# yerfor/Real3DPortrait

Hardware: NVIDIA H100
Metric: rendered frames/sec @512^2 (64^2 NeRF, 48 samples/ray) (higher is better)
Workload: dtype f32 render (decoder GEMMs: split-fp16 operands on wgmma, f32 accumulate, f32-grade results); SR f16 operands / f32 accumulate (wgmma)

## Files before the change

real3dportrait_b200/csrc/sr_tc.cu:

```cuda
#include "common.cuh"
#include "tc_prims.cuh"
#include <mutex>
#include <vector>
#include <type_traits>
#include <stdlib.h>

#ifndef R3DP_TC_DEBUG_TIMING
#define R3DP_TC_DEBUG_TIMING 0
#endif
namespace r3dp {
namespace tc {

constexpr int BM = 128, BN = 128, BK = 64;
constexpr float kSplitWeightScale = 1024.0f;


struct Taps {
    int n;
    int dy[9], dx[9], widx[9];
};
enum Mode { kStoreAct = 0, kStoreRaw = 1, kToRgbFinal = 2 };
struct ConvArgs {
    Taps taps;
    int k_chunks;
// ... 21 lines not shown
    Taps2 taps;
    int rows, oy_off, ox_off;
};
enum Mode2 { kActRgb = 3 };
struct Conv2Args {
    Phase2 ph[4];
    int n_phases, k_chunks, tiles_x, row_groups, n_blocks, n_images, total_units;
    int w_shared, mode;
    __half* out; int out_H, out_W, out_C, oy_mul, ox_mul;
    const float* bias; const float* wrgb; const float* brgb; const float* img_prev; float* img_out; int img_H, img_W;
    float act_slope, act_gain;
    int skip_same_res;
    const __half* residual;
    int out_clamp;
    uint8_t* img_out_u8;
    int split;
    int lo_off;
    int phase_mix;
    float acc_scale;
    unsigned long long* debug;
};


__device__ __forceinline__ float upsampled_skip(const float* __restrict__ ip, int h, int w, int Y, int X) {
    const float k4[4] = {0.25f, 0.75f, 0.75f, 0.25f};
    float acc = 0.f;
#pragma unroll
    for (int u = 0; u < 4; ++u) {
        const int zy = Y + u - 2;
        if (zy < 0 || (zy & 1) || (zy >> 1) >= h) continue;
        float rowv = 0.f;
#pragma unroll
        for (int v = 0; v < 4; ++v) {
            const int zx = X + v - 2;
            if (zx < 0 || (zx & 1) || (zx >> 1) >= w) continue;
            rowv = fmaf(k4[v], __ldg(ip + (size_t)(zy >> 1) * w + (zx >> 1)), rowv);
        }
        acc = fmaf(k4[u], rowv, acc);
    }
    return acc;
}

__device__ __forceinline__ float upsampled_skip_bf(const float* __restrict__ ip, int h, int w, int Y, int X) {
    const int y0 = (Y - 1) >> 1, x0 = (X - 1) >> 1;
    const float ky0 = (y0 >= 0 && y0 < h) ? ((Y & 1) ? 0.75f : 0.25f) : 0.f, ky1 = (y0 + 1 < h) ? ((Y & 1) ? 0.25f : 0.75f) : 0.f;
    const float kx0 = (x0 >= 0 && x0 < w) ? ((X & 1) ? 0.75f : 0.25f) : 0.f, kx1 = (x0 + 1 < w) ? ((X & 1) ? 0.25f : 0.75f) : 0.f;
    const int ya = min(max(y0, 0), h - 1), yb = min(y0 + 1, h - 1), xa = min(max(x0, 0), w - 1), xb = min(x0 + 1, w - 1);
    const float v00 = __ldg(ip + (size_t)ya * w + xa), v01 = __ldg(ip + (size_t)ya * w + xb);
    const float v10 = __ldg(ip + (size_t)yb * w + xa), v11 = __ldg(ip + (size_t)yb * w + xb);
    const float r0 = fmaf(kx1, v01, fmaf(kx0, v00, 0.f)), r1 = fmaf(kx1, v11, fmaf(kx0, v10, 0.f));
    return fmaf(ky1, r1, fmaf(ky0, r0, 0.f));
}

__device__ __forceinline__ float2 fma2(float2 a, float2 b, float2 c) { return make_float2(__fmaf_rn(a.x, b.x, c.x), __fmaf_rn(a.y, b.y, c.y)); }
__device__ __forceinline__ float2 mul2(float2 a, float2 b) { return make_float2(__fmul_rn(a.x, b.x), __fmul_rn(a.y, b.y)); }
__device__ __forceinline__ float2 add2(float2 a, float2 b) { return make_float2(__fadd_rn(a.x, b.x), __fadd_rn(a.y, b.y)); }

__device__ __forceinline__ uint4 pack_half8(const float* f) {
    __half2 h0 = __floats2half2_rn(f[0], f[1]), h1 = __floats2half2_rn(f[2], f[3]);
    __half2 h2 = __floats2half2_rn(f[4], f[5]), h3 = __floats2half2_rn(f[6], f[7]);
    uint4 pk;
    pk.x = *reinterpret_cast<uint32_t*>(&h0); pk.y = *reinterpret_cast<uint32_t*>(&h1);
    pk.z = *reinterpret_cast<uint32_t*>(&h2); pk.w = *reinterpret_cast<uint32_t*>(&h3);
    return pk;
}

__device__ __forceinline__ void store_half32(__half* dst, const float* f) {
    uint4* d4 = reinterpret_cast<uint4*>(dst);
#pragma unroll
    for (int v = 0; v < 4; ++v) {
        __half2 h0 = __floats2half2_rn(f[8 * v + 0], f[8 * v + 1]), h1 = __floats2half2_rn(f[8 * v + 2], f[8 * v + 3]);
        __half2 h2 = __floats2half2_rn(f[8 * v + 4], f[8 * v + 5]), h3 = __floats2half2_rn(f[8 * v + 6], f[8 * v + 7]);
        uint4 pk;
        pk.x = *reinterpret_cast<uint32_t*>(&h0); pk.y = *reinterpret_cast<uint32_t*>(&h1);
        pk.z = *reinterpret_cast<uint32_t*>(&h2); pk.w = *reinterpret_cast<uint32_t*>(&h3);
        d4[v] = pk;
    }
}

constexpr int kThreads3 = 384;
constexpr int B3_BYTES = BN * BK * 2;
constexpr int kStageRow = BN + 8;
template <int R> struct Cfg3 {
    static constexpr int NA = 4, NB = 4;
    static constexpr int TAIL = 8192;
    static constexpr int STAGE = 8 * 32 * 64;
    static constexpr int ACC = BM * kStageRow * 4;
    static constexpr int SMEM = NA * A2_SLOT + NB * B3_BYTES + 1024 + TAIL + STAGE + ACC;
};

template <int R, bool SPLIT>
__global__ void __launch_bounds__(kThreads3, 1) conv_tc3_kernel(const __grid_constant__ CUtensorMap tmA,
                                                               const __grid_constant__ CUtensorMap tmB, const Conv2Args a) {
    using C = Cfg3<R>;
    extern __shared__ uint8_t smem_raw[];
    uint8_t* smem = align_smem_1024(smem_raw);
    uint8_t* a_ring = smem;
    uint8_t* b_ring = smem + C::NA * A2_SLOT;
    uint8_t* tail = b_ring + C::NB * B3_BYTES;
    uint64_t* a_full = reinterpret_cast<uint64_t*>(tail);
    uint64_t* a_empty = a_full + C::NA;
    uint64_t* b_full = a_empty + C::NA;
    uint64_t* b_empty = b_full + C::NB;
    float* s_bias = reinterpret_cast<float*>(tail + 512);
    float* s_wrgb = s_bias + 256;
    float* s_part = s_wrgb + 768;
    uint4* s_stage = reinterpret_cast<uint4*>(tail + C::TAIL);
    float* s_acc = reinterpret_cast<float*>(tail + C::TAIL + C::STAGE);

    const int warp = threadIdx.x >> 5, lane = threadIdx.x & 31;
    const int units_per_image = a.n_phases * a.row_groups * a.tiles_x;

    if (threadIdx.x == 0) {
        for (int i = 0; i < C::NA; ++i) { mbar_init(&a_full[i], 1); mbar_init(&a_empty[i], 256); }
        for (int i = 0; i < C::NB; ++i) { mbar_init(&b_full[i], 1); mbar_init(&b_empty[i], 256); }
        asm volatile("fence.mbarrier_init.release.cluster;" ::: "memory");
        asm volatile("prefetch.tensormap [%0];" ::"l"(&tmA) : "memory");
        asm volatile("prefetch.tensormap [%0];" ::"l"(&tmB) : "memory");
    }
    if (warp >= 4) {
        const int t = threadIdx.x - 128;
        for (int e = t; e < a.n_blocks * BN && e < 256; e += 256) s_bias[e] = a.bias ? a.bias[e] : 0.f;
    }
    __syncthreads();

    const bool mix = a.phase_mix && a.n_phases > 1 && (a.tiles_x & 1) == 0;
    auto decode = [&](int unit, int& n, int& ph, int& row0, int& col0) {
        n = unit / units_per_image; int r = unit - n * units_per_image;
        const int xb = r % a.tiles_x; r /= a.tiles_x;
        int rg;
        if (mix) { rg = r / a.n_phases; ph = (r - rg * a.n_phases + rg) % a.n_phases; }
        else { rg = r % a.row_groups; ph = r / a.row_groups; }
        row0 = rg * R; col0 = xb * BM;
    };

    if (warp < 4) {
        if (warp == 0 && lane == 0) {
            uint32_t aq = 0, bq = 0;
            for (int unit = blockIdx.x; unit < a.total_units; unit += gridDim.x) {
                int n, ph, row0, col0; decode(unit, n, ph, row0, col0);
                const Taps2& tp = a.ph[ph].taps;
                const int DY = tp.ngroups;
                const int wn = a.w_shared ? 0 : n;
                const int K3 = SPLIT ? 3 * a.k_chunks : a.k_chunks;
                for (int nblk = 0; nblk < a.n_blocks; ++nblk)
                    for (int kq = 0; kq < K3; ++kq) {
                        const int kc = kq < 2 * a.k_chunks ? kq : kq - 2 * a.k_chunks;
                        const int kb = kq < a.k_chunks ? kq : kq - a.k_chunks;
                        for (int d = 0; d < DY; ++d) {
                            const int s_lo = d == 0 ? 0 : R - 1 + d, s_hi = R - 1 + d;
                            for (int s = s_lo; s <= s_hi; ++s, ++aq) {
                                const int slot = aq % C::NA;
                                mbar_wait(&a_empty[slot], ((aq / C::NA) & 1) ^ 1);
                                mbar_expect_tx(&a_full[slot], A2_BYTES);
                                tma_load_4d(a_ring + slot * A2_SLOT, &tmA, &a_full[slot], kc * BK, col0 - 1, row0 + tp.dy_min + s, n);
                            }
                            for (int t = tp.gstart[d]; t < tp.gstart[d + 1]; ++t, ++bq) {
                                const int slot = bq % C::NB;
                                mbar_wait(&b_empty[slot], ((bq / C::NB) & 1) ^ 1);
                                mbar_expect_tx(&b_full[slot], B3_BYTES);
                                tma_load_4d(b_ring + slot * B3_BYTES, &tmB, &b_full[slot], kb * BK, nblk * BN, tp.widx[t], wn);
                            }
                        }
                    }
            }
        }
    } else {
        const int wg = (warp >> 2) - 1;
        const int q = warp & 3, m = q * 32 + lane;
        const int cg = wg;
        const bool want_rgb = (a.mode == kToRgbFinal) || (a.mode == kActRgb);
        const int CW = a.n_blocks * BN;
        float brgb[3] = {0.f, 0.f, 0.f};
        if (want_rgb) { brgb[0] = a.brgb[0]; brgb[1] = a.brgb[1]; brgb[2] = a.brgb[2]; }
        int n_loaded = -1;
        uint32_t aq = 0, bq = 0;
        int pend_b = -1; uint32_t pend_a0 = 0, pend_an = 0;
        auto release_pending = [&]() {
            if (pend_b >= 0) mbar_arrive(&b_empty[pend_b]);
            for (uint32_t s = 0; s < pend_an; ++s) mbar_arrive(&a_empty[(pend_a0 + s) % C::NA]);
            pend_b = -1; pend_an = 0;
        };
        float acc[R][64];
        for (int unit = blockIdx.x; unit < a.total_units; unit += gridDim.x) {
            int n, ph, row0, col0; decode(unit, n, ph, row0, col0);
            const Phase2& P = a.ph[ph];
            const Taps2& tp = P.taps;
            const int DY = tp.ngroups, NS = R + DY - 1;
            const int wn = a.w_shared ? 0 : n;
            if (want_rgb && wn != n_loaded) {
                asm volatile("bar.sync 1, 256;" ::: "memory");
                for (int e = threadIdx.x - 128; e < 3 * CW; e += 256) s_wrgb[e] = a.wrgb[(size_t)wn * 3 * CW + e];
                asm volatile("bar.sync 1, 256;" ::: "memory");
                n_loaded = wn;
            }
            const int gcol = col0 + m, X = gcol * a.ox_mul + P.ox_off;
            float2 rgb2[R][3];
#pragma unroll
            for (int j = 0; j < R; ++j) { rgb2[j][0] = make_float2(0.f, 0.f); rgb2[j][1] = make_float2(0.f, 0.f); rgb2[j][2] = make_float2(0.f, 0.f); }
            float skipv[R][3];
#pragma unroll
            for (int j = 0; j < R; ++j) { skipv[j][0] = 0.f; skipv[j][1] = 0.f; skipv[j][2] = 0.f; }
            if (want_rgb && cg == 1 && a.img_prev) {
                if (a.skip_same_res) {
                    const int Xc = min(X, a.img_W - 1);
#pragma unroll
                    for (int j = 0; j < R; ++j) {
                        const int Yc = min((row0 + j) * a.oy_mul + P.oy_off, a.img_H - 1);
#pragma unroll
                        for (int c = 0; c < 3; ++c) skipv[j][c] = __ldg(a.img_prev + (((size_t)n * 3 + c) * a.img_H + Yc) * a.img_W + Xc);
                    }
                } else {
                    const int h = a.img_H / 2, w = a.img_W / 2;
                    const int x0 = (X - 1) >> 1;
                    const float kx0 = (x0 >= 0 && x0 < w) ? ((X & 1) ? 0.75f : 0.25f) : 0.f, kx1 = (x0 + 1 < w) ? ((X & 1) ? 0.25f : 0.75f) : 0.f;
                    const int xa = min(max(x0, 0), w - 1), xb = min(max(x0 + 1, 0), w - 1);
#pragma unroll
                    for (int j = 0; j < R; ++j) {
                        const int Y = (row0 + j) * a.oy_mul + P.oy_off, y0 = (Y - 1) >> 1;
                        const float ky0 = (y0 >= 0 && y0 < h) ? ((Y & 1) ? 0.75f : 0.25f) : 0.f;
                        const float ky1 = (y0 + 1 < h) ? ((Y & 1) ? 0.25f : 0.75f) : 0.f;
                        const int ya = min(max(y0, 0), h - 1), yb = min(max(y0 + 1, 0), h - 1);
#pragma unroll
                        for (int c = 0; c < 3; ++c) {
                            const float* ip = a.img_prev + ((size_t)n * 3 + c) * h * w;
                            const float v0 = __ldg(ip + ya * w + xa), v1 = __ldg(ip + ya * w + xb), v2 = __ldg(ip + yb * w + xa), v3 = __ldg(ip + yb * w + xb);
                            const float r0 = fmaf(kx1, v1, fmaf(kx0, v0, 0.f)), r1 = fmaf(kx1, v3, fmaf(kx0, v2, 0.f));
                            skipv[j][c] = fmaf(ky1, r1, fmaf(ky0, r0, 0.f));
                        }
                    }
                }
            }
            for (int nblk = 0; nblk < a.n_blocks; ++nblk) {
                const int K3 = SPLIT ? 3 * a.k_chunks : a.k_chunks;
                for (int kc = 0; kc < K3; ++kc) {
                    const uint32_t a_base = aq;
                    for (int d = 0; d < DY; ++d) {
                        const int s_lo = d == 0 ? 0 : R - 1 + d, s_hi = R - 1 + d;
                        for (int s = s_lo; s <= s_hi; ++s, ++aq) mbar_wait(&a_full[aq % C::NA], (aq / C::NA) & 1);
                        for (int t = tp.gstart[d]; t < tp.gstart[d + 1]; ++t, ++bq) {
                            const int bslot = bq % C::NB;
                            mbar_wait(&b_full[bslot], (bq / C::NB) & 1);
                            const uint64_t db = gmma_desc_sw128(smem_u32(b_ring + bslot * B3_BYTES));
                            const int sh = tp.shift[t];
                            const uint32_t first = (uint32_t)(kc | t);
                            uint64_t da[R];
#pragma unroll
                            for (int j = 0; j < R; ++j) da[j] = gmma_desc_sw128(smem_u32(a_ring + ((a_base + j + d) % C::NA) * A2_SLOT) + 128 * (64 * wg + sh));
                            wg_fence();
#pragma unroll
                            for (int k = 0; k < BK / 16; ++k) {
#pragma unroll
                                for (int j = 0; j < R; ++j) wgmma_m64n128k16(acc[j], da[j] + (uint64_t)(2 * k), db + (uint64_t)(2 * k), first | (uint32_t)k);
                            }
                            wg_commit();
                            wg_wait<1>();
                            release_pending();
                            pend_b = bslot;
                        }
                        if (d < DY - 1) { pend_a0 = a_base + d; pend_an = 1; }
                        else { pend_a0 = a_base + DY - 1; pend_an = (uint32_t)(NS - (DY - 1)); }
                    }
                }
                wg_wait<0>();
#pragma unroll
                for (int j = 0; j < R; ++j) wg_fence_acc<64>(acc[j]);
                release_pending();
#pragma unroll
                for (int j = 0; j < R; ++j) {
#pragma unroll
                    for (int i = 0; i < 64; i += 2)
                        *reinterpret_cast<float2*>(s_acc + (64 * wg + acc_row(i)) * kStageRow + acc_col(i)) = make_float2(acc[j][i], acc[j][i + 1]);
                    asm volatile("bar.sync 4, 256;" ::: "memory");
                    const int row = row0 + j;
                    const int Y = row * a.oy_mul + P.oy_off;
                    const bool row_ok = (row < P.rows) && (Y < a.out_H);
                    const bool in_img = row_ok && (X < a.out_W);
#pragma unroll 1
                    for (int c0 = cg * (BN / 2); c0 < (cg + 1) * (BN / 2); c0 += 32) {
                        float2 f2[16];
                        const float4* src = reinterpret_cast<const float4*>(s_acc + m * kStageRow + c0);
                        const float2 sc2 = make_float2(a.acc_scale, a.acc_scale);
#pragma unroll
                        for (int i = 0; i < 8; ++i) { const float4 v = src[i]; f2[2 * i] = make_float2(v.x, v.y); f2[2 * i + 1] = make_float2(v.z, v.w); }
                        if (a.mode == kStoreRaw) {
                            if (SPLIT) {
#pragma unroll
                                for (int i = 0; i < 16; ++i) f2[i] = mul2(f2[i], sc2);
                            }
                        } else {
                            const float2* b2 = reinterpret_cast<const float2*>(s_bias + nblk * BN + c0);
                            const float2 sl2 = make_float2(a.act_slope, a.act_slope), g2 = make_float2(a.act_gain, a.act_gain);
#pragma unroll
                            for (int i = 0; i < 16; ++i) {
                                const float2 v = SPLIT ? fma2(f2[i], sc2, b2[i]) : add2(f2[i], b2[i]);
                                const float2 t = mul2(v, sl2);
                                f2[i] = mul2(make_float2(fmaxf(v.x, t.x), fmaxf(v.y, t.y)), g2);
                            }
                        }
                        const float* f = reinterpret_cast<const float*>(f2);
                        if (a.mode != kToRgbFinal) {
                            uint4* st = s_stage + (warp - 4) * 128;
                            const int sw = (lane >> 1) & 3;
                            constexpr int passes = SPLIT ? 2 : 1;
#pragma unroll
                            for (int pass = 0; pass < passes; ++pass) {
                                if (pass == 0) {
#pragma unroll
                                    for (int v = 0; v < 4; ++v) st[lane * 4 + (v ^ sw)] = pack_half8(f + 8 * v);
                                } else {
#pragma unroll
                                    for (int v = 0; v < 4; ++v) {
                                        float lo[8];
#pragma unroll
                                        for (int e = 0; e < 8; ++e) lo[e] = f[8 * v + e] - __half2float(__float2half_rn(f[8 * v + e]));
                                        st[lane * 4 + (v ^ sw)] = pack_half8(lo);
                                    }
                                }
                                __syncwarp();
#pragma unroll
                                for (int i = 0; i < 4; ++i) {
                                    const int p = i * 8 + (lane >> 2), cch = lane & 3;
                                    uint4 pk = st[p * 4 + (cch ^ ((p >> 1) & 3))];
                                    const int Xp = (col0 + q * 32 + p) * a.ox_mul + P.ox_off;
                                    if (row_ok && Xp < a.out_W) {
                                        const size_t eo = ((size_t)n * a.out_H + Y) * a.out_W * a.out_C + nblk * BN + (size_t)Xp * a.out_C + c0 + cch * 8 + pass * a.lo_off;
                                        if (a.residual) {
                                            const uint4 rv = __ldg(reinterpret_cast<const uint4*>(a.residual + eo));
                                            __half2* ph = reinterpret_cast<__half2*>(&pk); const __half2* rh = reinterpret_cast<const __half2*>(&rv);
#pragma unroll
                                            for (int e = 0; e < 4; ++e) { const float2 x = __half22float2(ph[e]), r = __half22float2(rh[e]); ph[e] = __floats2half2_rn(x.x + r.x, x.y + r.y); }
                                        }
                                        *reinterpret_cast<uint4*>(a.out + eo) = pk;
                                    }
                                }
                                __syncwarp();
                            }
                        }
                        if (want_rgb) {
#pragma unroll
                            for (int c = 0; c < 3; ++c) {
                                const float4* w4 = reinterpret_cast<const float4*>(s_wrgb + c * CW + nblk * BN + c0);
                                float2 accr = rgb2[j][c];
#pragma unroll
                                for (int j4 = 0; j4 < 8; ++j4) {
                                    const float4 w = w4[j4];
                                    accr = fma2(f2[2 * j4], make_float2(w.x, w.y), accr);
                                    accr = fma2(f2[2 * j4 + 1], make_float2(w.z, w.w), accr);
                                }
                                rgb2[j][c] = accr;
                            }
                        }
                    }
                    if (want_rgb && nblk == a.n_blocks - 1) {
                        if (cg == 1) {
#pragma unroll
                            for (int c = 0; c < 3; ++c) s_part[(j * BM + m) * 3 + c] = (rgb2[j][c].x + rgb2[j][c].y) + skipv[j][c];
                        }
                        asm volatile("bar.sync 2, 256;" ::: "memory");
                        if (cg == 0) {
#pragma unroll
                            for (int c = 0; c < 3; ++c) rgb2[j][c].x = (rgb2[j][c].x + rgb2[j][c].y) + s_part[(j * BM + m) * 3 + c];
                        }
                        asm volatile("bar.sync 3, 256;" ::: "memory");
                    }
                    if (want_rgb && nblk == a.n_blocks - 1 && in_img && cg == 0) {
#pragma unroll
                        for (int c = 0; c < 3; ++c) {
                            float v = rgb2[j][c].x + brgb[c];
                            if (a.out_clamp) v = fminf(fmaxf(v, -1.0f), 1.0f);
                            if (a.img_out_u8)
                                a.img_out_u8[(((size_t)n * a.img_H + Y) * a.img_W + X) * 3 + c] =
                                    (uint8_t)(int)__fmul_rn(__fmul_rn(__fadd_rn(v, 1.0f), 0.5f), 255.0f);
                            else
                                a.img_out[(((size_t)n * 3 + c) * a.img_H + Y) * a.img_W + X] = v;
                        }
                    }
                    asm volatile("bar.sync 5, 256;" ::: "memory");
                }
            }
        }
    }
}

__device__ __forceinline__ void split_half(float v, __half& hi, __half& lo) {
    hi = __float2half_rn(v);
    lo = __float2half_rn(v - __half2float(hi));
}

__global__ void pack_weights_kernel(const float* __restrict__ wf, int Nw, int O, int I, int Ip, int split, __half* __restrict__ out) {
    const long long idx = (long long)blockIdx.x * blockDim.x + threadIdx.x;
    const long long total = (long long)Nw * 9 * O * Ip;
    if (idx >= total) return;
    const int i = (int)(idx % Ip); const int o = (int)((idx / Ip) % O); const int t = (int)((idx / ((long long)Ip * O)) % 9);
    const int nw = (int)(idx / ((long long)Ip * O * 9));
    const float v = i < I ? wf[(((size_t)nw * O + o) * I + i) * 9 + t] : 0.f;
    if (!split) { out[idx] = __float2half_rn(v); return; }
    __half hi, lo;
    split_half(v * kSplitWeightScale, hi, lo);
    const size_t row = (idx / Ip) * (size_t)(2 * Ip);
    out[row + i] = hi; out[row + Ip + i] = lo;
}

__global__ void resize_to_nhwc_f16_kernel(const float* __restrict__ x, int N, int C, int h, int w, int size, int Cp, int split, __half* __restrict__ y) {
    const long long idx = (long long)blockIdx.x * blockDim.x + threadIdx.x;
    if (idx >= (long long)N * size * size * Cp) return;
    const int c = (int)(idx % Cp); const int ox = (int)((idx / Cp) % size); const int oy = (int)((idx / ((long long)Cp * size)) % size);
    const int n = (int)(idx / ((long long)Cp * size * size));
    float v = 0.f;
    if (c < C) {
        const float sy = fmaxf(((float)oy + 0.5f) * ((float)h / (float)size) - 0.5f, 0.f);
        const float sx = fmaxf(((float)ox + 0.5f) * ((float)w / (float)size) - 0.5f, 0.f);
        const int y0 = min((int)sy, h - 1), x0 = min((int)sx, w - 1), y1 = min(y0 + 1, h - 1), x1 = min(x0 + 1, w - 1);
        const float ty = sy - (float)y0, tx = sx - (float)x0;
        const float* p = x + ((size_t)n * C + c) * h * w;
        const float r0 = p[y0 * w + x0] * (1.f - ty) + p[y1 * w + x0] * ty;
        const float r1 = p[y0 * w + x1] * (1.f - ty) + p[y1 * w + x1] * ty;
        v = r0 * (1.f - tx) + r1 * tx;
    }
    if (!split) { y[idx] = __float2half_rn(v); return; }
    __half hi, lo;
    split_half(v, hi, lo);
    const size_t pix = (idx / Cp) * (size_t)(2 * Cp);
    y[pix + c] = hi; y[pix + Cp + c] = lo;
}

constexpr int kEdgeRows = 16, kEdgeRowsSplit = 16, kEdgeCo = 32;
__global__ void __launch_bounds__(256) upconv_edge_kernel(const __half* __restrict__ x, const __half* __restrict__ wp, int H, int W, int Cp, int O,
                                                          int w_shared, __half* __restrict__ yb) {
    extern __shared__ __align__(16) uint8_t edge_smem[];
    __half* s_x = reinterpret_cast<__half*>(edge_smem);
// ... 255 lines not shown
        if (cudaGetDriverEntryPoint("cuTensorMapEncodeTiled", &p, cudaEnableDefault, &q) == cudaSuccess && q == cudaDriverEntryPointSuccess)
            fn = reinterpret_cast<EncodeTiledFn>(p);
    });
    return fn;
}

static int make_map_4d_box(CUtensorMap* m, const void* ptr, uint64_t d0, uint64_t d1, uint64_t d2, uint64_t d3, uint32_t box1);
static int make_map_4d(CUtensorMap* m, const void* ptr, uint64_t d0, uint64_t d1, uint64_t d2, uint64_t d3, uint32_t box1) {
    return make_map_4d_box(m, ptr, d0, d1, d2, d3, box1);
}
static int make_map_4d_box(CUtensorMap* m, const void* ptr, uint64_t d0, uint64_t d1, uint64_t d2, uint64_t d3, uint32_t box1) {
    EncodeTiledFn fn = encode_fn();
    R3DP_REQUIRE(fn != nullptr, "cuTensorMapEncodeTiled is not available from the driver");
    cuuint64_t dims[4] = {d0, d1, d2, d3};
    cuuint64_t strides[3] = {d0 * 2, d0 * d1 * 2, d0 * d1 * d2 * 2};
    cuuint32_t box[4] = {64, box1, 1, 1};
    cuuint32_t estr[4] = {1, 1, 1, 1};
    CUresult r = fn(m, CU_TENSOR_MAP_DATA_TYPE_FLOAT16, 4, const_cast<void*>(ptr), dims, strides, box, estr, CU_TENSOR_MAP_INTERLEAVE_NONE,
                    CU_TENSOR_MAP_SWIZZLE_128B, CU_TENSOR_MAP_L2_PROMOTION_L2_256B, CU_TENSOR_MAP_FLOAT_OOB_FILL_NONE);
    R3DP_REQUIRE(r == CUDA_SUCCESS, "cuTensorMapEncodeTiled failed with CUresult %d (dims %llu x %llu x %llu x %llu)", (int)r,
                 (unsigned long long)d0, (unsigned long long)d1, (unsigned long long)d2, (unsigned long long)d3);
    return 0;
}

static int make_map_fir(CUtensorMap* m, const void* ptr, uint64_t d0, uint64_t d1, uint64_t d2, uint64_t d3, uint32_t box_rows) {
    EncodeTiledFn fn = encode_fn();
    R3DP_REQUIRE(fn != nullptr, "cuTensorMapEncodeTiled is not available from the driver");
    cuuint64_t dims[4] = {d0, d1, d2, d3};
    cuuint64_t strides[3] = {d0 * 2, d0 * d1 * 2, d0 * d1 * d2 * 2};
    cuuint32_t box[4] = {64, (cuuint32_t)FIR_BW, box_rows, 1};
    cuuint32_t estr[4] = {1, 1, 1, 1};
    CUresult r = fn(m, CU_TENSOR_MAP_DATA_TYPE_FLOAT16, 4, const_cast<void*>(ptr), dims, strides, box, estr, CU_TENSOR_MAP_INTERLEAVE_NONE,
                    CU_TENSOR_MAP_SWIZZLE_128B, CU_TENSOR_MAP_L2_PROMOTION_L2_256B, CU_TENSOR_MAP_FLOAT_OOB_FILL_NONE);
    R3DP_REQUIRE(r == CUDA_SUCCESS, "cuTensorMapEncodeTiled (FIR) failed with CUresult %d", (int)r);
    return 0;
}

static int launch_conv2(const void* x, int N, int H, int W, int Cp, const void* wp, int Nw, int O, const ConvArgs& a1, cudaStream_t st);
static int launch_upconv2(const void* x, int N, int H, int W, int Cp, const void* wp, int Nw, int O, __half* yb, const float* bias, int split, cudaStream_t st);
static int launch_conv(const void* x, int N, int H, int W, int Cp, const void* wp, int Nw, int O, ConvArgs a, cudaStream_t st) {
    return launch_conv2(x, N, H, W, Cp, wp, Nw, O, a, st);
}

struct ConvProf { bool on = false; std::vector<cudaEvent_t> ev; size_t used = 0; };
static ConvProf g_prof;
static void prof_mark(cudaStream_t st) {
    if (!g_prof.on) return;
    if (g_prof.used == g_prof.ev.size()) { cudaEvent_t e; if (cudaEventCreate(&e) != cudaSuccess) return; g_prof.ev.push_back(e); }
    cudaEventRecord(g_prof.ev[g_prof.used++], st);
}

static unsigned long long* g_debug_buf = nullptr;
static int g_debug_launch = 0;
constexpr int kConvRows = 1;

template <int R, bool SPLIT>
static int launch_conv3_rs(const CUtensorMap& tmA, const CUtensorMap& tmB, Conv2Args a, int max_rows, cudaStream_t st) {
    using C = Cfg3<R>;
    R3DP_CUDA(cudaFuncSetAttribute(conv_tc3_kernel<R, SPLIT>, cudaFuncAttributeMaxDynamicSharedMemorySize, C::SMEM));
    a.debug = g_debug_buf ? g_debug_buf + 24 * (g_debug_launch++ % 32) : nullptr;
    a.row_groups = (max_rows + R - 1) / R;
    a.total_units = a.n_images * a.n_phases * a.row_groups * a.tiles_x;
    const int grid = a.total_units < sm_count() ? a.total_units : sm_count();
    prof_mark(st);
    conv_tc3_kernel<R, SPLIT><<<grid, kThreads3, C::SMEM, st>>>(tmA, tmB, a);
    R3DP_LAUNCH_CHECK();
    prof_mark(st);
    count_launches(1);
    return 0;
}
template <int R>
static int launch_conv3_r(const CUtensorMap& tmA, const CUtensorMap& tmB, const Conv2Args& a, int max_rows, cudaStream_t st) {
    return a.split ? launch_conv3_rs<R, true>(tmA, tmB, a, max_rows, st) : launch_conv3_rs<R, false>(tmA, tmB, a, max_rows, st);
}

static void fill_taps2(Taps2& t2, const Taps& t) {
    int order[9], n = t.n;
    for (int i = 0; i < n; ++i) order[i] = i;
    for (int i = 0; i < n; ++i)
        for (int j = i + 1; j < n; ++j) {
            const int a = order[i], b = order[j];
            if (t.dy[b] < t.dy[a] || (t.dy[b] == t.dy[a] && t.dx[b] < t.dx[a])) { order[i] = b; order[j] = a; }
        }
    int dy_min = 99;
    for (int i = 0; i < n; ++i) if (t.dy[i] < dy_min) dy_min = t.dy[i];
    t2.n = n; t2.dy_min = dy_min; t2.ngroups = 0;
    int last = -99;
    for (int i = 0; i < n; ++i) {
        const int o = order[i];
        if (t.dy[o] != last) { t2.gstart[t2.ngroups++] = i; last = t.dy[o]; }
        t2.dyi[i] = t.dy[o] - dy_min; t2.shift[i] = t.dx[o] + 1; t2.widx[i] = t.widx[o];
    }
    t2.gstart[t2.ngroups] = n;
}

static int run_conv2(const void* x, int N, int H, int W, int Cp, const void* wp, int Nw, int O, Conv2Args& a, int max_rows, cudaStream_t st, int n_taps = 9) {
    CUtensorMap tmA, tmB;
    const uint64_t Cphys = (uint64_t)Cp * (a.split ? 2 : 1);
    if (make_map_4d_box(&tmA, x, Cphys, (uint64_t)W, (uint64_t)H, (uint64_t)N, A2_ROWS)) return 1;
    if (make_map_4d_box(&tmB, wp, Cphys, (uint64_t)O, (uint64_t)n_taps, (uint64_t)Nw, BN)) return 1;
    if (a.split) { R3DP_REQUIRE(a.residual == nullptr, "conv_tc3: the residual epilogue is not built for split operands"); a.acc_scale = 1.0f / kSplitWeightScale; a.lo_off = a.out_C; a.out_C *= 2; }
    else { a.acc_scale = 1.0f; a.lo_off = 0; }
    a.k_chunks = Cp / BK; a.tiles_x = W / BM; a.n_blocks = O / BN; a.n_images = N; a.w_shared = (Nw == 1);
    { static int mixv = -1; if (mixv < 0) { const char* e = getenv("R3DP_TC_MIX"); mixv = (e && e[0] == '0') ? 0 : 1; } a.phase_mix = mixv; }
    if (a.act_gain == 0.f) { a.act_slope = 0.2f; a.act_gain = 1.4142135623730951f; }
    R3DP_REQUIRE(a.n_blocks >= 1 && a.n_blocks <= 2, "conv_tc3: 128 or 256 output channels");
    return launch_conv3_r<kConvRows>(tmA, tmB, a, max_rows, st);
}

static int launch_conv2(const void* x, int N, int H, int W, int Cp, const void* wp, int Nw, int O, const ConvArgs& a1, cudaStream_t st) {
    Conv2Args a = {};
    a.n_phases = 1;
    fill_taps2(a.ph[0].taps, a1.taps);
    a.ph[0].rows = a1.rows; a.ph[0].oy_off = a1.oy_off; a.ph[0].ox_off = a1.ox_off;
    a.mode = a1.mode; a.out = a1.out; a.out_H = a1.out_H; a.out_W = a1.out_W; a.out_C = a1.out_C; a.oy_mul = a1.oy_mul; a.ox_mul = a1.ox_mul;
    a.bias = a1.bias; a.wrgb = a1.wrgb; a.brgb = a1.brgb; a.img_prev = a1.img_prev; a.img_out = a1.img_out; a.img_H = a1.out_H; a.img_W = a1.out_W;
    a.out_clamp = a1.out_clamp; a.img_out_u8 = a1.img_out_u8; a.split = a1.split;
    return run_conv2(x, N, H, W, Cp, wp, Nw, O, a, a1.rows, st);
}

static int launch_upconv2(const void* x, int N, int H, int W, int Cp, const void* wp, int Nw, int O, __half* yb, const float* bias, int split, cudaStream_t st) {
    Conv2Args a = {};
    a.n_phases = 4; a.split = split;
    for (int pa = 0; pa < 2; ++pa)
        for (int pb = 0; pb < 2; ++pb) {
            Taps t = {};
            for (int ky = pa; ky < 3; ky += 2)
                for (int kx = pb; kx < 3; kx += 2) { const int i = t.n++; t.dy[i] = -(ky >> 1); t.dx[i] = -(kx >> 1); t.widx[i] = ky * 3 + kx; }
            Phase2& P = a.ph[pa * 2 + pb];
            fill_taps2(P.taps, t);
            P.rows = pa ? H : H + 1; P.oy_off = pa; P.ox_off = pb;
        }
    a.mode = kStoreRaw; a.out = yb; a.out_H = 2 * H + 1; a.out_W = 2 * W + 1; a.out_C = O; a.oy_mul = a.ox_mul = 2; a.bias = bias;
    return run_conv2(x, N, H, W, Cp, wp, Nw, O, a, H + 1, st);
}

}
}

using namespace r3dp;
using namespace r3dp::tc;

static int pack_weights_impl(const float* wf, int Nw, int O, int I, void* packed_f16, int split, r3dp_stream_t stream) {
    R3DP_REQUIRE(wf && packed_f16, "sr_tc_pack_weights: null pointer");
    R3DP_REQUIRE(Nw > 0 && O > 0 && I > 0, "sr_tc_pack_weights: bad shape");
    const int Ip = (I + 63) / 64 * 64;
    const long long total = (long long)Nw * 9 * O * Ip;
    pack_weights_kernel<<<(unsigned)((total + 255) / 256), 256, 0, as_stream(stream)>>>(wf, Nw, O, I, Ip, split, reinterpret_cast<__half*>(packed_f16));
    R3DP_LAUNCH_CHECK();
    count_launches(1);
    return 0;
}
extern "C" int r3dp_sr_tc_pack_weights(const float* wf, int Nw, int O, int I, void* packed_f16, r3dp_stream_t stream) { return pack_weights_impl(wf, Nw, O, I, packed_f16, 0, stream); }
extern "C" int r3dp_sr_tcx_pack_weights(const float* wf, int Nw, int O, int I, void* packed_f16, r3dp_stream_t stream) { return pack_weights_impl(wf, Nw, O, I, packed_f16, 1, stream); }

static int input_impl(const float* x, int N, int C, int h, int w, int size, void* y_f16, int split, r3dp_stream_t stream) {
    R3DP_REQUIRE(x && y_f16, "sr_tc_input: null pointer");
    R3DP_REQUIRE(N > 0 && C > 0 && h > 0 && w > 0 && size >= h && size >= w, "sr_tc_input: up-scaling (or copy) only");
    const int Cp = (C + 63) / 64 * 64;
    const long long total = (long long)N * size * size * Cp;
// ... 493 lines not shown
```

real3dportrait_b200/csrc/tc_prims.cuh:

```cuda
#pragma once
#include <cuda.h>
#include <cuda_fp16.h>
#include <stdint.h>

namespace r3dp {
namespace tc {

__device__ __forceinline__ uint32_t smem_u32(const void* p) { return (uint32_t)__cvta_generic_to_shared(p); }
__device__ __forceinline__ uint8_t* align_smem_1024(uint8_t* p) { return p + ((1024u - (smem_u32(p) & 1023u)) & 1023u); }
__device__ __forceinline__ void mbar_init(uint64_t* b, uint32_t count) {
    asm volatile("mbarrier.init.shared::cta.b64 [%0], %1;" ::"r"(smem_u32(b)), "r"(count));
}
__device__ __forceinline__ void mbar_expect_tx(uint64_t* b, uint32_t bytes) {
    asm volatile("mbarrier.arrive.expect_tx.shared::cta.b64 _, [%0], %1;" ::"r"(smem_u32(b)), "r"(bytes) : "memory");
}
__device__ __forceinline__ void mbar_arrive(uint64_t* b) {
    asm volatile("mbarrier.arrive.shared::cta.b64 _, [%0];" ::"r"(smem_u32(b)) : "memory");
}
__device__ __forceinline__ void mbar_wait(uint64_t* b, uint32_t parity) {
    asm volatile(
        "{\n\t.reg .pred p;\n\t"
        "WAIT_LOOP:\n\t"
        "mbarrier.try_wait.parity.shared::cta.b64 p, [%0], %1;\n\t"
        "@p bra DONE;\n\t"
        "bra WAIT_LOOP;\n\t"
        "DONE:\n\t}" ::"r"(smem_u32(b)), "r"(parity) : "memory");
}
__device__ __forceinline__ void tma_load_4d(void* dst, const CUtensorMap* map, uint64_t* bar, int c0, int c1, int c2, int c3) {
    asm volatile(
        "cp.async.bulk.tensor.4d.shared::cluster.global.mbarrier::complete_tx::bytes [%0], [%1, {%3, %4, %5, %6}], [%2];"
        ::"r"(smem_u32(dst)), "l"(map), "r"(smem_u32(bar)), "r"(c0), "r"(c1), "r"(c2), "r"(c3) : "memory");
}
__device__ __forceinline__ bool elect_one() {
    uint32_t pred;
    asm volatile("{\n\t.reg .pred P1;\n\telect.sync _|P1, 0xffffffff;\n\tselp.b32 %0, 1, 0, P1;\n\t}" : "=r"(pred));
    return pred != 0;
}

__device__ __forceinline__ void wg_fence() { asm volatile("wgmma.fence.sync.aligned;" ::: "memory"); }
__device__ __forceinline__ void wg_commit() { asm volatile("wgmma.commit_group.sync.aligned;" ::: "memory"); }
template <int N>
__device__ __forceinline__ void wg_wait() { asm volatile("wgmma.wait_group.sync.aligned %0;" ::"n"(N) : "memory"); }
template <int NR>
__device__ __forceinline__ void wg_fence_acc(float* d) {
#pragma unroll
    for (int i = 0; i < NR; ++i) asm volatile("" : "+f"(d[i])::"memory");
}
__device__ __forceinline__ int acc_row(int i) { return ((threadIdx.x >> 5) & 3) * 16 + ((threadIdx.x & 31) >> 2) + 8 * ((i >> 1) & 1); }
__device__ __forceinline__ int acc_col(int i) { return 8 * (i >> 2) + 2 * (threadIdx.x & 3) + (i & 1); }

__device__ __forceinline__ void wgmma_m64n48k16(float* d, uint64_t desc_a, uint64_t desc_b, uint32_t accumulate) {
    asm volatile(
        "{\n\t.reg .pred p;\n\t"
        "setp.ne.b32 p, %26, 0;\n\t"
        "wgmma.mma_async.sync.aligned.m64n48k16.f32.f16.f16 "
        "{%0,%1,%2,%3,%4,%5,%6,%7,%8,%9,%10,%11,%12,%13,%14,%15,%16,%17,%18,%19,%20,%21,%22,%23}, %24, %25, p, 1, 1, 0, 0;\n\t}"
        : "+f"(d[0]), "+f"(d[1]), "+f"(d[2]), "+f"(d[3]), "+f"(d[4]), "+f"(d[5]), "+f"(d[6]), "+f"(d[7]), "+f"(d[8]), "+f"(d[9]), "+f"(d[10]), "+f"(d[11]), "+f"(d[12]), "+f"(d[13]), "+f"(d[14]), "+f"(d[15]), "+f"(d[16]), "+f"(d[17]), "+f"(d[18]), "+f"(d[19]), "+f"(d[20]), "+f"(d[21]), "+f"(d[22]), "+f"(d[23])
        : "l"(desc_a), "l"(desc_b), "r"(accumulate));
}

__device__ __forceinline__ void wgmma_m64n64k16(float* d, uint64_t desc_a, uint64_t desc_b, uint32_t accumulate) {
    asm volatile(
        "{\n\t.reg .pred p;\n\t"
        "setp.ne.b32 p, %34, 0;\n\t"
        "wgmma.mma_async.sync.aligned.m64n64k16.f32.f16.f16 "
        "{%0,%1,%2,%3,%4,%5,%6,%7,%8,%9,%10,%11,%12,%13,%14,%15,%16,%17,%18,%19,%20,%21,%22,%23,%24,%25,%26,%27,%28,%29,%30,%31}, %32, %33, p, 1, 1, 0, 0;\n\t}"
        : "+f"(d[0]), "+f"(d[1]), "+f"(d[2]), "+f"(d[3]), "+f"(d[4]), "+f"(d[5]), "+f"(d[6]), "+f"(d[7]), "+f"(d[8]), "+f"(d[9]), "+f"(d[10]), "+f"(d[11]), "+f"(d[12]), "+f"(d[13]), "+f"(d[14]), "+f"(d[15]), "+f"(d[16]), "+f"(d[17]), "+f"(d[18]), "+f"(d[19]), "+f"(d[20]), "+f"(d[21]), "+f"(d[22]), "+f"(d[23]), "+f"(d[24]), "+f"(d[25]), "+f"(d[26]), "+f"(d[27]), "+f"(d[28]), "+f"(d[29]), "+f"(d[30]), "+f"(d[31])
        : "l"(desc_a), "l"(desc_b), "r"(accumulate));
}

__device__ __forceinline__ void wgmma_m64n128k16(float* d, uint64_t desc_a, uint64_t desc_b, uint32_t accumulate) {
    asm volatile(
        "{\n\t.reg .pred p;\n\t"
        "setp.ne.b32 p, %66, 0;\n\t"
        "wgmma.mma_async.sync.aligned.m64n128k16.f32.f16.f16 "
        "{%0,%1,%2,%3,%4,%5,%6,%7,%8,%9,%10,%11,%12,%13,%14,%15,%16,%17,%18,%19,%20,%21,%22,%23,%24,%25,%26,%27,%28,%29,%30,%31,%32,%33,%34,%35,%36,%37,%38,%39,%40,%41,%42,%43,%44,%45,%46,%47,%48,%49,%50,%51,%52,%53,%54,%55,%56,%57,%58,%59,%60,%61,%62,%63}, %64, %65, p, 1, 1, 0, 0;\n\t}"
        : "+f"(d[0]), "+f"(d[1]), "+f"(d[2]), "+f"(d[3]), "+f"(d[4]), "+f"(d[5]), "+f"(d[6]), "+f"(d[7]), "+f"(d[8]), "+f"(d[9]), "+f"(d[10]), "+f"(d[11]), "+f"(d[12]), "+f"(d[13]), "+f"(d[14]), "+f"(d[15]), "+f"(d[16]), "+f"(d[17]), "+f"(d[18]), "+f"(d[19]), "+f"(d[20]), "+f"(d[21]), "+f"(d[22]), "+f"(d[23]), "+f"(d[24]), "+f"(d[25]), "+f"(d[26]), "+f"(d[27]), "+f"(d[28]), "+f"(d[29]), "+f"(d[30]), "+f"(d[31]), "+f"(d[32]), "+f"(d[33]), "+f"(d[34]), "+f"(d[35]), "+f"(d[36]), "+f"(d[37]), "+f"(d[38]), "+f"(d[39]), "+f"(d[40]), "+f"(d[41]), "+f"(d[42]), "+f"(d[43]), "+f"(d[44]), "+f"(d[45]), "+f"(d[46]), "+f"(d[47]), "+f"(d[48]), "+f"(d[49]), "+f"(d[50]), "+f"(d[51]), "+f"(d[52]), "+f"(d[53]), "+f"(d[54]), "+f"(d[55]), "+f"(d[56]), "+f"(d[57]), "+f"(d[58]), "+f"(d[59]), "+f"(d[60]), "+f"(d[61]), "+f"(d[62]), "+f"(d[63])
        : "l"(desc_a), "l"(desc_b), "r"(accumulate));
}


__device__ __forceinline__ uint64_t gmma_desc_sw128(uint32_t saddr) {
    uint64_t d = 0;
    d |= (uint64_t)((saddr & 0x3ffff) >> 4);
    d |= (uint64_t)1 << 16;
// ... 7 lines not shown
```

real3dportrait_b200/engine.py:

```python
from __future__ import annotations

import contextlib
import os
from typing import Callable, Dict, Optional

import torch

from . import _capi as capi
from .renderer import PlanesCL
from .synthesis import RenderHead


@contextlib.contextmanager
def gpu_local_cpus(device_index: int = 0, report: Optional[dict] = None):
    old = None
    info = {'gpu_numa_node': None, 'pinned_to_gpu_node': False, 'reason': ''}
    try:
        pr = torch.cuda.get_device_properties(device_index)
        addr = f'{pr.pci_domain_id:04x}:{pr.pci_bus_id:02x}:{pr.pci_device_id:02x}.0'
        try:
            info['gpu_numa_node'] = int(open(f'/sys/bus/pci/devices/{addr}/numa_node').read().strip())
        except Exception:
            pass
        txt = open(f'/sys/bus/pci/devices/{addr}/local_cpulist').read().strip()
# ... 298 lines not shown
                dst.copy_(src)
            self.prepare([hp['stage'][k]])
            hp['in_free'][k].record(cur); hp['out_free'][k].record(cur)
        stage = hp['stage'][k]
        with torch.cuda.stream(hp['copy_in']):
            hp['copy_in'].wait_event(hp['in_free'][k])
            for dst, src in zip(stage, hosts):
                dst.copy_(src, non_blocking=True)
            hp['in_ready'][k].record(hp['copy_in'])
        cur.wait_event(hp['in_ready'][k])
        out = self.step(*stage)
        self.wait_gather()
        hp['in_free'][k].record(cur)
        cur.wait_event(hp['out_free'][k])
        mine = out[self.rank * self.batch:(self.rank + 1) * self.batch] if out.shape[0] > self.batch else out
        hp['out'][k].copy_(mine, non_blocking=True)
        hp['out_ready'][k].record(cur)
        with torch.cuda.stream(hp['copy_out']):
            hp['copy_out'].wait_event(hp['out_ready'][k])
            h_out.copy_(hp['out'][k], non_blocking=True)
            hp['out_free'][k].record(hp['copy_out'])

    def sync_host(self) -> None:
        hp = self._host_pipeline()
        hp['copy_in'].synchronize(); hp['copy_out'].synchronize(); torch.cuda.current_stream().synchronize()

    def static_inputs(self):
        return self.s_in

    def profile_steps(self, inputs: Callable[[int], tuple], first: int, steps: int) -> Dict:
        capi.PROF = capi.Profiler()
        self.step(*inputs(first))
        torch.cuda.synchronize()
        capi.PROF = capi.Profiler()
        L = capi.lib()
        tc = self.head.superresolution.sr_mode in ('tc', 'tc_exact')
        if tc:
            L.r3dp_sr_tc_prof(1)
        a, b = torch.cuda.Event(enable_timing=True), torch.cuda.Event(enable_timing=True)
        a.record()
        for i in range(steps):
            self.step(*inputs(first + i))
        b.record()
        torch.cuda.synchronize()
        stages = capi.PROF.totals()
        capi.PROF = None
        conv_ms, conv_n = None, 0
        if tc:
            import ctypes as C
            ms, n = C.c_float(0), C.c_int(0)
            capi.check(L.r3dp_sr_tc_prof_read(C.byref(ms), C.byref(n)))
            L.r3dp_sr_tc_prof(0)
            conv_ms, conv_n = float(ms.value), int(n.value)
        kernel = 'conv_tc3_kernel<1> (wgmma implicit-GEMM conv)' if tc else 'conv_taps_kernel (fp32 CUDA-core direct conv)'
        return {'stages': stages, 'sr_conv_ms': stages.get('sr_conv', float('nan')), 'total_ms': a.elapsed_time(b), 'sr_kernel': kernel,
                'conv_kernel_ms': conv_ms, 'conv_launches': conv_n}
```

Before: 1724.

## Process two output rows per conv tile with register-direct epilogue and setmaxnreg

The conv kernel now handles two output rows per work unit (R=2), so each weight/activation halo load feeds more wgmma work. The fp32 accumulator staging in shared memory is removed: bias, activation, fp16 packing and the toRGB dot products run directly on the wgmma fragment registers, and the toRGB partials are reduced with warp shuffles instead of shared-memory exchanges and named barriers. Producer warps give up registers and consumer warps take more through setmaxnreg, which makes room for the doubled accumulators. The TMA rings deepen from 4 to 6 stages, using the shared memory freed by dropping the accumulator staging buffer. The risks are register pressure or spills at 232 regs and wasted rows when the row count is odd.

```diff
diff --git a/real3dportrait_b200/csrc/sr_tc.cu b/real3dportrait_b200/csrc/sr_tc.cu
--- a/real3dportrait_b200/csrc/sr_tc.cu
+++ b/real3dportrait_b200/csrc/sr_tc.cu
@@ -97,19 +97,6 @@
     return fmaf(ky1, r1, fmaf(ky0, r0, 0.f));
 }
 
-__device__ __forceinline__ float2 fma2(float2 a, float2 b, float2 c) { return make_float2(__fmaf_rn(a.x, b.x, c.x), __fmaf_rn(a.y, b.y, c.y)); }
-__device__ __forceinline__ float2 mul2(float2 a, float2 b) { return make_float2(__fmul_rn(a.x, b.x), __fmul_rn(a.y, b.y)); }
-__device__ __forceinline__ float2 add2(float2 a, float2 b) { return make_float2(__fadd_rn(a.x, b.x), __fadd_rn(a.y, b.y)); }
-
-__device__ __forceinline__ uint4 pack_half8(const float* f) {
-    __half2 h0 = __floats2half2_rn(f[0], f[1]), h1 = __floats2half2_rn(f[2], f[3]);
-    __half2 h2 = __floats2half2_rn(f[4], f[5]), h3 = __floats2half2_rn(f[6], f[7]);
-    uint4 pk;
-    pk.x = *reinterpret_cast<uint32_t*>(&h0); pk.y = *reinterpret_cast<uint32_t*>(&h1);
-    pk.z = *reinterpret_cast<uint32_t*>(&h2); pk.w = *reinterpret_cast<uint32_t*>(&h3);
-    return pk;
-}
-
 __device__ __forceinline__ void store_half32(__half* dst, const float* f) {
     uint4* d4 = reinterpret_cast<uint4*>(dst);
 #pragma unroll
@@ -123,21 +110,23 @@
     }
 }
 
+constexpr int kConvRows = 2;
 constexpr int kThreads3 = 384;
+constexpr int kProducerRegs = 40, kConsumerRegs = 232;
 constexpr int B3_BYTES = BN * BK * 2;
-constexpr int kStageRow = BN + 8;
-template <int R> struct Cfg3 {
-    static constexpr int NA = 4, NB = 4;
+struct Cfg3 {
+    static constexpr int NA = 6, NB = 6;
     static constexpr int TAIL = 8192;
-    static constexpr int STAGE = 8 * 32 * 64;
-    static constexpr int ACC = BM * kStageRow * 4;
-    static constexpr int SMEM = NA * A2_SLOT + NB * B3_BYTES + 1024 + TAIL + STAGE + ACC;
+    static constexpr int STAGE = 8 * 8 * BN * 2;
+    static constexpr int SMEM = NA * A2_SLOT + NB * B3_BYTES + 1024 + TAIL + STAGE;
 };
-
-template <int R, bool SPLIT>
+static_assert(Cfg3::SMEM <= 227 * 1024, "conv_tc3: shared memory over the sm_90 per-block limit");
+
+template <bool SPLIT>
 __global__ void __launch_bounds__(kThreads3, 1) conv_tc3_kernel(const __grid_constant__ CUtensorMap tmA,
                                                                const __grid_constant__ CUtensorMap tmB, const Conv2Args a) {
-    using C = Cfg3<R>;
+    using C = Cfg3;
+    constexpr int R = kConvRows;
     extern __shared__ uint8_t smem_raw[];
     uint8_t* smem = align_smem_1024(smem_raw);
     uint8_t* a_ring = smem;
@@ -149,9 +138,7 @@
     uint64_t* b_empty = b_full + C::NB;
     float* s_bias = reinterpret_cast<float*>(tail + 512);
     float* s_wrgb = s_bias + 256;
-    float* s_part = s_wrgb + 768;
     uint4* s_stage = reinterpret_cast<uint4*>(tail + C::TAIL);
-    float* s_acc = reinterpret_cast<float*>(tail + C::TAIL + C::STAGE);
 
     const int warp = threadIdx.x >> 5, lane = threadIdx.x & 31;
     const int units_per_image = a.n_phases * a.row_groups * a.tiles_x;
@@ -180,6 +167,7 @@
     };
 
     if (warp < 4) {
+        setmaxnreg_dec<kProducerRegs>();
         if (warp == 0 && lane == 0) {
             uint32_t aq = 0, bq = 0;
             for (int unit = blockIdx.x; unit < a.total_units; unit += gridDim.x) {
@@ -211,9 +199,9 @@
             }
         }
     } else {
+        setmaxnreg_inc<kConsumerRegs>();
         const int wg = (warp >> 2) - 1;
-        const int q = warp & 3, m = q * 32 + lane;
-        const int cg = wg;
+        const int quad = lane & 3, pix = 64 * wg + 16 * (warp & 3) + (lane >> 2);
         const bool want_rgb = (a.mode == kToRgbFinal) || (a.mode == kActRgb);
         const int CW = a.n_blocks * BN;
         float brgb[3] = {0.f, 0.f, 0.f};
@@ -239,14 +227,17 @@
                 asm volatile("bar.sync 1, 256;" ::: "memory");
                 n_loaded = wn;
             }
-            const int gcol = col0 + m, X = gcol * a.ox_mul + P.ox_off;
-            float2 rgb2[R][3];
-#pragma unroll
-            for (int j = 0; j < R; ++j) { rgb2[j][0] = make_float2(0.f, 0.f); rgb2[j][1] = make_float2(0.f, 0.f); rgb2[j][2] = make_float2(0.f, 0.f); }
+            const bool rgb_lane = want_rgb && quad < 2;
+            const int X = (col0 + pix + 8 * quad) * a.ox_mul + P.ox_off;
+            float rgb[R][2][3];
+#pragma unroll
+            for (int j = 0; j < R; ++j)
+#pragma unroll
+                for (int h = 0; h < 2; ++h) { rgb[j][h][0] = 0.f; rgb[j][h][1] = 0.f; rgb[j][h][2] = 0.f; }
             float skipv[R][3];
 #pragma unroll
             for (int j = 0; j < R; ++j) { skipv[j][0] = 0.f; skipv[j][1] = 0.f; skipv[j][2] = 0.f; }
-            if (want_rgb && cg == 1 && a.img_prev) {
+            if (rgb_lane && a.img_prev) {
                 if (a.skip_same_res) {
                     const int Xc = min(X, a.img_W - 1);
 #pragma unroll
@@ -311,108 +302,103 @@
 #pragma unroll
                 for (int j = 0; j < R; ++j) wg_fence_acc<64>(acc[j]);
                 release_pending();
-#pragma unroll
-                for (int j = 0; j < R; ++j) {
-#pragma unroll
-                    for (int i = 0; i < 64; i += 2)
-                        *reinterpret_cast<float2*>(s_acc + (64 * wg + acc_row(i)) * kStageRow + acc_col(i)) = make_float2(acc[j][i], acc[j][i + 1]);
-                    asm volatile("bar.sync 4, 256;" ::: "memory");
-                    const int row = row0 + j;
-                    const int Y = row * a.oy_mul + P.oy_off;
-                    const bool row_ok = (row < P.rows) && (Y < a.out_H);
-                    const bool in_img = row_ok && (X < a.out_W);
-#pragma unroll 1
-                    for (int c0 = cg * (BN / 2); c0 < (cg + 1) * (BN / 2); c0 += 32) {
-                        float2 f2[16];
-                        const float4* src = reinterpret_cast<const float4*>(s_acc + m * kStageRow + c0);
-                        const float2 sc2 = make_float2(a.acc_scale, a.acc_scale);
-#pragma unroll
-                        for (int i = 0; i < 8; ++i) { const float4 v = src[i]; f2[2 * i] = make_float2(v.x, v.y); f2[2 * i + 1] = make_float2(v.z, v.w); }
-                        if (a.mode == kStoreRaw) {
-                            if (SPLIT) {
-#pragma unroll
-                                for (int i = 0; i < 16; ++i) f2[i] = mul2(f2[i], sc2);
-                            }
-                        } else {
-                            const float2* b2 = reinterpret_cast<const float2*>(s_bias + nblk * BN + c0);
-                            const float2 sl2 = make_float2(a.act_slope, a.act_slope), g2 = make_float2(a.act_gain, a.act_gain);
-#pragma unroll
-                            for (int i = 0; i < 16; ++i) {
-                                const float2 v = SPLIT ? fma2(f2[i], sc2, b2[i]) : add2(f2[i], b2[i]);
-                                const float2 t = mul2(v, sl2);
-                                f2[i] = mul2(make_float2(fmaxf(v.x, t.x), fmaxf(v.y, t.y)), g2);
-                            }
-                        }
-                        const float* f = reinterpret_cast<const float*>(f2);
-                        if (a.mode != kToRgbFinal) {
-                            uint4* st = s_stage + (warp - 4) * 128;
-                            const int sw = (lane >> 1) & 3;
-                            constexpr int passes = SPLIT ? 2 : 1;
-#pragma unroll
-                            for (int pass = 0; pass < passes; ++pass) {
-                                if (pass == 0) {
-#pragma unroll
-                                    for (int v = 0; v < 4; ++v) st[lane * 4 + (v ^ sw)] = pack_half8(f + 8 * v);
-                                } else {
-#pragma unroll
-                                    for (int v = 0; v < 4; ++v) {
-                                        float lo[8];
-#pragma unroll
-                                        for (int e = 0; e < 8; ++e) lo[e] = f[8 * v + e] - __half2float(__float2half_rn(f[8 * v + e]));
-                                        st[lane * 4 + (v ^ sw)] = pack_half8(lo);
-                                    }
+                if (a.mode == kStoreRaw) {
+                    if (SPLIT) {
+#pragma unroll
+                        for (int j = 0; j < R; ++j)
+#pragma unroll
+                            for (int i = 0; i < 64; ++i) acc[j][i] = __fmul_rn(acc[j][i], a.acc_scale);
+                    }
+                } else {
+#pragma unroll
+                    for (int i = 0; i < 16; ++i) {
+                        const float2 b2 = *reinterpret_cast<const float2*>(s_bias + nblk * BN + 8 * i + 2 * quad);
+#pragma unroll
+                        for (int j = 0; j < R; ++j)
+#pragma unroll
+                            for (int h = 0; h < 2; ++h)
+#pragma unroll
+                                for (int e = 0; e < 2; ++e) {
+                                    float& x = acc[j][4 * i + 2 * h + e];
+                                    const float b = e ? b2.y : b2.x;
+                                    const float v = SPLIT ? __fmaf_rn(x, a.acc_scale, b) : __fadd_rn(x, b);
+                                    x = __fmul_rn(fmaxf(v, __fmul_rn(v, a.act_slope)), a.act_gain);
+                                }
+                    }
+                }
+                if (a.mode != kToRgbFinal) {
+                    uint4* st = s_stage + (warp - 4) * 128;
+                    uint32_t* st32 = reinterpret_cast<uint32_t*>(st);
+                    const int sr = lane >> 2;
+                    constexpr int passes = SPLIT ? 2 : 1;
+#pragma unroll
+                    for (int j = 0; j < R; ++j) {
+                        const int row = row0 + j, Y = row * a.oy_mul + P.oy_off;
+                        const bool row_ok = (row < P.rows) && (Y < a.out_H);
+#pragma unroll
+                        for (int pass = 0; pass < passes; ++pass)
+#pragma unroll
+                            for (int h = 0; h < 2; ++h) {
+#pragma unroll
+                                for (int i = 0; i < 16; ++i) {
+                                    float x0 = acc[j][4 * i + 2 * h], x1 = acc[j][4 * i + 2 * h + 1];
+                                    if (pass) { x0 = x0 - __half2float(__float2half_rn(x0)); x1 = x1 - __half2float(__float2half_rn(x1)); }
+                                    const __half2 hv = __floats2half2_rn(x0, x1);
+                                    st32[sr * 64 + (i ^ sr) * 4 + quad] = *reinterpret_cast<const uint32_t*>(&hv);
                                 }
                                 __syncwarp();
 #pragma unroll
-                                for (int i = 0; i < 4; ++i) {
-                                    const int p = i * 8 + (lane >> 2), cch = lane & 3;
-                                    uint4 pk = st[p * 4 + (cch ^ ((p >> 1) & 3))];
-                                    const int Xp = (col0 + q * 32 + p) * a.ox_mul + P.ox_off;
+                                for (int it = 0; it < 4; ++it) {
+                                    const int p = 2 * it + (lane >> 4), cch = lane & 15;
+                                    uint4 pk = st[p * 16 + (cch ^ p)];
+                                    const int Xp = (col0 + pix - sr + p + 8 * h) * a.ox_mul + P.ox_off;
                                     if (row_ok && Xp < a.out_W) {
-                                        const size_t eo = ((size_t)n * a.out_H + Y) * a.out_W * a.out_C + nblk * BN + (size_t)Xp * a.out_C + c0 + cch * 8 + pass * a.lo_off;
+                                        const size_t eo = ((size_t)n * a.out_H + Y) * a.out_W * a.out_C + nblk * BN + (size_t)Xp * a.out_C + cch * 8 + pass * a.lo_off;
                                         if (a.residual) {
                                             const uint4 rv = __ldg(reinterpret_cast<const uint4*>(a.residual + eo));
-                                            __half2* ph = reinterpret_cast<__half2*>(&pk); const __half2* rh = reinterpret_cast<const __half2*>(&rv);
-#pragma unroll
-                                            for (int e = 0; e < 4; ++e) { const float2 x = __half22float2(ph[e]), r = __half22float2(rh[e]); ph[e] = __floats2half2_rn(x.x + r.x, x.y + r.y); }
+                                            __half2* ph2 = reinterpret_cast<__half2*>(&pk); const __half2* rh = reinterpret_cast<const __half2*>(&rv);
+#pragma unroll
+                                            for (int e = 0; e < 4; ++e) { const float2 x = __half22float2(ph2[e]), r = __half22float2(rh[e]); ph2[e] = __floats2half2_rn(x.x + r.x, x.y + r.y); }
                                         }
                                         *reinterpret_cast<uint4*>(a.out + eo) = pk;
                                     }
                                 }
                                 __syncwarp();
                             }
+                    }
+                }
+                if (want_rgb) {
+#pragma unroll
+                    for (int c = 0; c < 3; ++c)
+#pragma unroll
+                        for (int i = 0; i < 16; ++i) {
+                            const float2 w2 = *reinterpret_cast<const float2*>(s_wrgb + c * CW + nblk * BN + 8 * i + 2 * quad);
+#pragma unroll
+                            for (int j = 0; j < R; ++j)
+#pragma unroll
+                                for (int h = 0; h < 2; ++h)
+                                    rgb[j][h][c] = fmaf(acc[j][4 * i + 2 * h + 1], w2.y, fmaf(acc[j][4 * i + 2 * h], w2.x, rgb[j][h][c]));
                         }
-                        if (want_rgb) {
-#pragma unroll
-                            for (int c = 0; c < 3; ++c) {
-                                const float4* w4 = reinterpret_cast<const float4*>(s_wrgb + c * CW + nblk * BN + c0);
-                                float2 accr = rgb2[j][c];
-#pragma unroll
-                                for (int j4 = 0; j4 < 8; ++j4) {
-                                    const float4 w = w4[j4];
-                                    accr = fma2(f2[2 * j4], make_float2(w.x, w.y), accr);
-                                    accr = fma2(f2[2 * j4 + 1], make_float2(w.z, w.w), accr);
-                                }
-                                rgb2[j][c] = accr;
-                            }
+                }
+            }
+            if (want_rgb) {
+#pragma unroll
+                for (int j = 0; j < R; ++j)
+#pragma unroll
+                    for (int h = 0; h < 2; ++h)
+#pragma unroll
+                        for (int c = 0; c < 3; ++c) {
+                            rgb[j][h][c] += __shfl_xor_sync(0xffffffffu, rgb[j][h][c], 1);
+                            rgb[j][h][c] += __shfl_xor_sync(0xffffffffu, rgb[j][h][c], 2);
                         }
-                    }
-                    if (want_rgb && nblk == a.n_blocks - 1) {
-                        if (cg == 1) {
-#pragma unroll
-                            for (int c = 0; c < 3; ++c) s_part[(j * BM + m) * 3 + c] = (rgb2[j][c].x + rgb2[j][c].y) + skipv[j][c];
-                        }
-                        asm volatile("bar.sync 2, 256;" ::: "memory");
-                        if (cg == 0) {
-#pragma unroll
-                            for (int c = 0; c < 3; ++c) rgb2[j][c].x = (rgb2[j][c].x + rgb2[j][c].y) + s_part[(j * BM + m) * 3 + c];
-                        }
-                        asm volatile("bar.sync 3, 256;" ::: "memory");
-                    }
-                    if (want_rgb && nblk == a.n_blocks - 1 && in_img && cg == 0) {
+                if (rgb_lane) {
+#pragma unroll
+                    for (int j = 0; j < R; ++j) {
+                        const int row = row0 + j, Y = row * a.oy_mul + P.oy_off;
+                        if (row >= P.rows || Y >= a.out_H || X >= a.out_W) continue;
 #pragma unroll
                         for (int c = 0; c < 3; ++c) {
-                            float v = rgb2[j][c].x + brgb[c];
+                            float v = ((quad ? rgb[j][1][c] : rgb[j][0][c]) + skipv[j][c]) + brgb[c];
                             if (a.out_clamp) v = fminf(fmaxf(v, -1.0f), 1.0f);
                             if (a.img_out_u8)
                                 a.img_out_u8[(((size_t)n * a.img_H + Y) * a.img_W + X) * 3 + c] =
@@ -421,7 +407,6 @@
                                 a.img_out[(((size_t)n * 3 + c) * a.img_H + Y) * a.img_W + X] = v;
                         }
                     }
-                    asm volatile("bar.sync 5, 256;" ::: "memory");
                 }
             }
         }
@@ -783,26 +768,19 @@
 
 static unsigned long long* g_debug_buf = nullptr;
 static int g_debug_launch = 0;
-constexpr int kConvRows = 1;
-
-template <int R, bool SPLIT>
-static int launch_conv3_rs(const CUtensorMap& tmA, const CUtensorMap& tmB, Conv2Args a, int max_rows, cudaStream_t st) {
-    using C = Cfg3<R>;
-    R3DP_CUDA(cudaFuncSetAttribute(conv_tc3_kernel<R, SPLIT>, cudaFuncAttributeMaxDynamicSharedMemorySize, C::SMEM));
+template <bool SPLIT>
+static int launch_conv3_s(const CUtensorMap& tmA, const CUtensorMap& tmB, Conv2Args a, int max_rows, cudaStream_t st) {
+    R3DP_CUDA(cudaFuncSetAttribute(conv_tc3_kernel<SPLIT>, cudaFuncAttributeMaxDynamicSharedMemorySize, Cfg3::SMEM));
     a.debug = g_debug_buf ? g_debug_buf + 24 * (g_debug_launch++ % 32) : nullptr;
-    a.row_groups = (max_rows + R - 1) / R;
+    a.row_groups = (max_rows + kConvRows - 1) / kConvRows;
     a.total_units = a.n_images * a.n_phases * a.row_groups * a.tiles_x;
     const int grid = a.total_units < sm_count() ? a.total_units : sm_count();
     prof_mark(st);
-    conv_tc3_kernel<R, SPLIT><<<grid, kThreads3, C::SMEM, st>>>(tmA, tmB, a);
+    conv_tc3_kernel<SPLIT><<<grid, kThreads3, Cfg3::SMEM, st>>>(tmA, tmB, a);
     R3DP_LAUNCH_CHECK();
     prof_mark(st);
     count_launches(1);
     return 0;
-}
-template <int R>
-static int launch_conv3_r(const CUtensorMap& tmA, const CUtensorMap& tmB, const Conv2Args& a, int max_rows, cudaStream_t st) {
-    return a.split ? launch_conv3_rs<R, true>(tmA, tmB, a, max_rows, st) : launch_conv3_rs<R, false>(tmA, tmB, a, max_rows, st);
 }
 
 static void fill_taps2(Taps2& t2, const Taps& t) {
@@ -836,7 +814,7 @@
     { static int mixv = -1; if (mixv < 0) { const char* e = getenv("R3DP_TC_MIX"); mixv = (e && e[0] == '0') ? 0 : 1; } a.phase_mix = mixv; }
     if (a.act_gain == 0.f) { a.act_slope = 0.2f; a.act_gain = 1.4142135623730951f; }
     R3DP_REQUIRE(a.n_blocks >= 1 && a.n_blocks <= 2, "conv_tc3: 128 or 256 output channels");
-    return launch_conv3_r<kConvRows>(tmA, tmB, a, max_rows, st);
+    return a.split ? launch_conv3_s<true>(tmA, tmB, a, max_rows, st) : launch_conv3_s<false>(tmA, tmB, a, max_rows, st);
 }
 
 static int launch_conv2(const void* x, int N, int H, int W, int Cp, const void* wp, int Nw, int O, const ConvArgs& a1, cudaStream_t st) {
diff --git a/real3dportrait_b200/csrc/tc_prims.cuh b/real3dportrait_b200/csrc/tc_prims.cuh
--- a/real3dportrait_b200/csrc/tc_prims.cuh
+++ b/real3dportrait_b200/csrc/tc_prims.cuh
@@ -31,6 +31,10 @@
         "cp.async.bulk.tensor.4d.shared::cluster.global.mbarrier::complete_tx::bytes [%0], [%1, {%3, %4, %5, %6}], [%2];"
         ::"r"(smem_u32(dst)), "l"(map), "r"(smem_u32(bar)), "r"(c0), "r"(c1), "r"(c2), "r"(c3) : "memory");
 }
+template <int N>
+__device__ __forceinline__ void setmaxnreg_dec() { asm volatile("setmaxnreg.dec.sync.aligned.u32 %0;" ::"n"(N)); }
+template <int N>
+__device__ __forceinline__ void setmaxnreg_inc() { asm volatile("setmaxnreg.inc.sync.aligned.u32 %0;" ::"n"(N)); }
 __device__ __forceinline__ bool elect_one() {
     uint32_t pred;
     asm volatile("{\n\t.reg .pred P1;\n\telect.sync _|P1, 0xffffffff;\n\tselp.b32 %0, 1, 0, P1;\n\t}" : "=r"(pred));
diff --git a/real3dportrait_b200/engine.py b/real3dportrait_b200/engine.py
--- a/real3dportrait_b200/engine.py
+++ b/real3dportrait_b200/engine.py
@@ -374,6 +374,6 @@
             capi.check(L.r3dp_sr_tc_prof_read(C.byref(ms), C.byref(n)))
             L.r3dp_sr_tc_prof(0)
             conv_ms, conv_n = float(ms.value), int(n.value)
-        kernel = 'conv_tc3_kernel<1> (wgmma implicit-GEMM conv)' if tc else 'conv_taps_kernel (fp32 CUDA-core direct conv)'
+        kernel = 'conv_tc3_kernel (wgmma implicit-GEMM conv, 2-row tiles)' if tc else 'conv_taps_kernel (fp32 CUDA-core direct conv)'
         return {'stages': stages, 'sr_conv_ms': stages.get('sr_conv', float('nan')), 'total_ms': a.elapsed_time(b), 'sr_kernel': kernel,
                 'conv_kernel_ms': conv_ms, 'conv_launches': conv_n}
```

Result: faster. 2120 (median of 6 runs) (+22.9%).
